# DakeQQ/Text-to-Speech-TTS-ONNX

Hardware: AMD Instinct MI355X
Metric: audio_seconds_per_second (higher is better)
Workload: dtype f32

## Files before the change

text-to-speech-tts-onnx_amd/csrc/gemm_x3d.hip:

```cpp
#include "common.h"
#include "mfma.h"
#include "gemm_epilogue.h"
#include "x3_split.h"
#include "lds_dma.h"
#include <type_traits>
#include <algorithm>

namespace mi {

typedef float f32x4 __attribute__((ext_vector_type(4)));

template <int TW> struct X3dGeom {
    static constexpr int TM = 144, MB = 3;
    static constexpr int KG = TW == 64 ? 2 : 1;
    static constexpr int WNS = KG == 2 ? 2 : 4;
    static constexpr int WNW = TW / WNS, NB = WNW / 16;
#ifndef X3D_S128
#define X3D_S128 1
#endif
    static constexpr int S = TW == 192 ? 1 : TW == 128 ? X3D_S128 : 2;
    static constexpr int WSTEP = TW == 128 ? X3D_S128 : 1;
    static constexpr int R = TW == 64 ? 6 : TW == 128 ? 4 : 3;
    static constexpr int LB = R / S - 1;
    static constexpr int A_PLANE = TM * 64, B_PLANE = TW * 64;
    static constexpr int A_BYTES = 2 * A_PLANE, CH = A_BYTES + 2 * B_PLANE;
    static constexpr int PC = CH / 1024, P = S * PC;
    static constexpr int NHI = (P + 11) / 12, NHIW = P - 12 * (NHI - 1);
    static constexpr int NCB = TW / 64, NRB = 5, BLK = 2176;
    static constexpr int STG = NRB * NCB * BLK * 4, RING = R * CH;
    static constexpr int LNT = RING > STG ? RING : STG;
    static constexpr int SMEM = LNT + 2 * 160 * 4;
    static_assert(SMEM <= 163840, "x3d: LDS");
};

template <int OFF> __device__ __forceinline__ void x3d_lds_rd128(f16x8& d, unsigned a) {
#if defined(__HIP_DEVICE_COMPILE__)
    asm volatile("ds_read_b128 %0, %1 offset:%2" : "=v"(d) : "v"(a), "n"(OFF) : "memory");
#endif
}
template <int OFF, int N> struct X3dRd {
    static __device__ __forceinline__ void go(f16x8 (&dst)[N], unsigned a) {
        X3dRd<OFF, N - 1>::go(reinterpret_cast<f16x8 (&)[N - 1]>(dst), a);
        x3d_lds_rd128<OFF + (N - 1) * 1024>(dst[N - 1], a);
    }
};
template <int OFF> struct X3dRd<OFF, 1> {
    static __device__ __forceinline__ void go(f16x8 (&dst)[1], unsigned a) { x3d_lds_rd128<OFF>(dst[0], a); }
};
template <int N, int I = 0, typename F> __device__ __forceinline__ void x3d_unroll(F&& f) {
    if constexpr (I < N) { f(std::integral_constant<int, I>{}); x3d_unroll<N, I + 1>(f); }
}
template <int TW, bool FOLD, int EPK>
__global__ __launch_bounds__(768) void linear_x3d_kernel(const ConvGemmDev p) {
    using G = X3dGeom<TW>;
    using Frag = f16x8;
    constexpr int MB = G::MB, NB = G::NB;
    __shared__ __attribute__((aligned(1024))) unsigned char smem[G::SMEM];
    (void)smem;
#if defined(__HIP_DEVICE_COMPILE__)
    const int tid = threadIdx.x, lane = tid & 63;
    const int wave = __builtin_amdgcn_readfirstlane(tid >> 6);
    const int per = (int)gridDim.x >> 3;
    const int u = ((int)blockIdx.x & 7) * per + ((int)blockIdx.x >> 3);
    const int RGn = p.Tm, CGn = p.Tn, band = p.RT;
    if (u >= RGn * CGn) return;
    const int bi = u / (band * CGn);
    const int rem = u - bi * band * CGn;
    const int bh = min(band, RGn - bi * band);
    const int cg = rem / bh, rg = bi * band + rem - cg * bh;
    const int m0 = rg * G::TM, n0 = cg * TW;
    const int nch = p.K >> 5;

    const int kg = G::KG == 2 ? wave / 6 : 0;
    const int w6 = G::KG == 2 ? wave - kg * 6 : wave;
    const int wm = w6 / G::WNS, wn = w6 - wm * G::WNS;

    const int bytesA = (int)((long)((p.M + 127) >> 7) * nch * 16384), bytesB = (int)((long)((p.N + 127) >> 7) * nch * 16384);
    const unsigned smem_lds = lds_addr(smem);
    const int voff = lane * 16;
    constexpr int OOB = 0x7fffff00;
    int pc_gbase[G::NHI], pc_cs[G::NHI];
    unsigned pc_lofs[G::NHI];
    __amdgpu_buffer_rsrc_t pc_rs[G::NHI];
#pragma unroll
    for (int i = 0; i < G::NHI; ++i) {
        const int q = wave + 12 * i;
        const int cs = q / G::PC, r = q - cs * G::PC;
        const bool isA = r < 18;
        const int rr = isA ? r : r - 18;
        const int gpp = isA ? 9 : TW / 16;
        const int plane = rr / gpp, g16 = rr - plane * gpp;
        const int row = (isA ? m0 : n0) + 16 * g16;
        pc_cs[i] = cs;
        pc_rs[i] = buf_rsrc(isA ? p.x : p.w3, isA ? bytesA : bytesB);
        pc_gbase[i] = __builtin_amdgcn_readfirstlane((row >> 7) * nch * 16384 + plane * 8192 + (row & 127) * 64);
        pc_lofs[i] = (unsigned)__builtin_amdgcn_readfirstlane(isA ? plane * G::A_PLANE + g16 * 1024 : G::A_BYTES + plane * G::B_PLANE + g16 * 1024);
    }
    const bool hi_wave = wave < G::NHIW;
    auto issue_piece = [&](int t, auto I_) __attribute__((always_inline)) {
        constexpr int i = decltype(I_)::value;
        if constexpr (i < G::NHI) {
            if (i == G::NHI - 1 && !hi_wave) return;
            const int chunk = t * G::S + pc_cs[i];
            const int soff = __builtin_amdgcn_readfirstlane(chunk < nch ? pc_gbase[i] + chunk * 16384 : OOB);
            const unsigned dst = __builtin_amdgcn_readfirstlane(smem_lds + (unsigned)((chunk % G::R) * G::CH) + pc_lofs[i]);
            dma16_buf(pc_rs[i], (int)((unsigned)voff + (unsigned)soff), dst);
        }
    };
    auto issue_batch = [&](int t) __attribute__((always_inline)) {
        x3d_unroll<G::NHI>([&](auto I_) __attribute__((always_inline)) { issue_piece(t, I_); });
    };
    auto wait_batches = [&](auto NB_) __attribute__((always_inline)) {
        constexpr int n = decltype(NB_)::value;
        if (hi_wave) wait_vm<n * G::NHI>(); else wait_vm<n * (G::NHI - 1)>();
    };

    const int fi = lane & 15, fs = lane >> 4;
    const int sig = (0x1320 >> (4 * (fi >> 2))) & 3;
    const unsigned f_lane = (unsigned)((4 * sig + (fi & 3)) * 64 + ((fs ^ sig) << 4));
    const unsigned fa_off = (unsigned)(wm * 48 * 64) + f_lane;
    const unsigned fb_off = (unsigned)(G::A_BYTES + wn * G::WNW * 64) + f_lane;
    Frag a_lo[MB], a_hi[MB], b_lo[NB], b_hi[NB];
    f32x4 acc0[MB][NB], acc1[MB][NB];
#pragma unroll
    for (int i = 0; i < MB; ++i)
#pragma unroll
        for (int j = 0; j < NB; ++j) { acc0[i][j] = f32x4{0.f, 0.f, 0.f, 0.f}; acc1[i][j] = f32x4{0.f, 0.f, 0.f, 0.f}; }
    auto rd_a = [&](unsigned a, auto PL, Frag (&dst)[MB]) __attribute__((always_inline)) {
        constexpr int pl = decltype(PL)::value;
        X3dRd<pl * G::A_PLANE, MB>::go(dst, a);
    };
    auto rd_b = [&](unsigned b, auto PL, Frag (&dst)[NB]) __attribute__((always_inline)) {
        constexpr int pl = decltype(PL)::value;
        X3dRd<pl * G::B_PLANE, NB>::go(dst, b);
    };
    using P0 = std::integral_constant<int, 0>;
    using P1 = std::integral_constant<int, 1>;
    auto mma = [&](const Frag (&a)[MB], const Frag (&b)[NB], f32x4 (&c)[MB][NB]) __attribute__((always_inline)) {
#pragma unroll
        for (int i = 0; i < MB; ++i)
#pragma unroll
            for (int j = 0; j < NB; ++j) c[i][j] = __builtin_amdgcn_mfma_f32_16x16x32_f16(a[i], b[j], c[i][j], 0, 0, 0);
    };
#define X3D_SB() __builtin_amdgcn_sched_barrier(0)

    const int NJ = nch / G::KG;
#pragma unroll
    for (int t = 0; t <= G::LB; ++t) issue_batch(t);
    float* lnt = reinterpret_cast<float*>(smem + G::LNT);
    constexpr bool CONSUMER = FOLD && (EPK == 1 || EPK == 2);
    if constexpr (CONSUMER) {
        if (wave < G::NRB && p.ln_stats_in) {
            float rs, mr;
            ln_rows32(p, (long)p.m_off + m0 + wave * 32, (long)p.m_off + p.M - 1, lane & 31, lane >> 5, rs, mr);
            if (lane < 32) { lnt[wave * 32 + lane] = rs; lnt[160 + wave * 32 + lane] = mr; }
        }
    }
    wait_batches(std::integral_constant<int, G::LB>{});
    __builtin_amdgcn_s_barrier();
    {
        const unsigned s0 = smem_lds + (unsigned)((kg % G::R) * G::CH);
        rd_a(s0 + fa_off, P1{}, a_lo); rd_b(s0 + fb_off, P0{}, b_hi); rd_a(s0 + fa_off, P0{}, a_hi); rd_b(s0 + fb_off, P1{}, b_lo);
    }
    auto chunk = [&](int j, auto BAR_) __attribute__((always_inline)) {
        constexpr bool BAR = decltype(BAR_)::value;
        wait_lgkm<MB + NB>();
        X3D_SB(); mma(a_lo, b_hi, acc1); X3D_SB();
        const int jn = j + 1;
        const int ts = jn / G::WSTEP;
        if constexpr (BAR) {
            wait_batches(std::integral_constant<int, G::LB - 1>{});
            wait_lgkm<0>();
            __builtin_amdgcn_s_barrier();
        }
        const unsigned sn = smem_lds + (unsigned)(((jn * G::KG + kg) % G::R) * G::CH);
        rd_a(sn + fa_off, P1{}, a_lo);
        wait_lgkm<MB>();
        X3D_SB();
        x3d_unroll<MB * NB>([&](auto IDX_) __attribute__((always_inline)) {
            constexpr int idx = decltype(IDX_)::value, i = idx / NB, jj = idx % NB;
            acc0[i][jj] = __builtin_amdgcn_mfma_f32_16x16x32_f16(a_hi[i], b_hi[jj], acc0[i][jj], 0, 0, 0);
            if constexpr (BAR) issue_piece(ts + G::LB, IDX_);
            X3D_SB();
        });
        rd_b(sn + fb_off, P0{}, b_hi);
        X3D_SB(); mma(a_hi, b_lo, acc1); X3D_SB();
        rd_a(sn + fa_off, P0{}, a_hi); rd_b(sn + fb_off, P1{}, b_lo);
    };
    static_assert(G::NHI <= MB * NB, "x3d: a batch's pieces ride on the MFMAs of phase 1");
    for (int j = 0; j < NJ; j += G::WSTEP) {
        if constexpr (G::WSTEP == 2) chunk(j, std::false_type{});
        chunk(j + G::WSTEP - 1, std::true_type{});
    }
#undef X3D_SB
    wait_vm<0>();
    wait_lgkm<0>();
    __builtin_amdgcn_s_barrier();
    if (p.dbg & 4) return;

    float* stg = reinterpret_cast<float*>(smem);
    {
        const int rq = 4 * ((0x1320 >> (4 * (lane >> 4))) & 3);
        const int cq = 4 * ((0x1320 >> (4 * ((lane & 15) >> 2))) & 3) + (lane & 3);
        auto put = [&](bool add) __attribute__((always_inline)) {
#pragma unroll
            for (int i = 0; i < MB; ++i) {
                const int row = wm * 48 + i * 16 + rq;
#pragma unroll
                for (int j = 0; j < NB; ++j) {
                    const int col = wn * G::WNW + j * 16 + cq;
                    float* d = stg + ((row >> 5) * G::NCB + (col >> 6)) * G::BLK + (row & 31) * 64 + (col & 63);
#pragma unroll
                    for (int r = 0; r < 4; ++r) {
                        const float v = __builtin_fmaf(acc1[i][j][r], 0x1p-11f, acc0[i][j][r]);
                        d[r * 64] = add ? d[r * 64] + v : v;
                    }
                }
            }
        };
        if (G::KG == 1 || kg == 0) put(false);
        __syncthreads();
        if constexpr (G::KG == 2) {
            if (kg == 1) put(true);
            __syncthreads();
        }
    }
    const int lr = lane & 31, lk = lane >> 5;
    const int m_end = min(p.M, m0 + G::TM);
    constexpr bool HALVES = EPK == 3 && (G::NRB * G::NCB * G::BLK + 12 * 1024) * 4 <= G::LNT;
    if constexpr (HALVES) {
        float* half_stage = stg + G::NRB * G::NCB * G::BLK;
        for (int u = wave; u < G::NRB * G::NCB * 2; u += 12) {
            const int b = u >> 1, hf = u & 1;
            const int rb = b / G::NCB, cb = b - rb * G::NCB;
            if (m0 + rb * 32 >= m_end) continue;
            const float* blk = stg + b * G::BLK + hf * 32;
            f32x16 h1[1][1];
#pragma unroll
            for (int r = 0; r < 16; ++r) {
                const float t = blk[((r & 3) + 8 * (r >> 2) + 4 * lk) * 64 + lr];
                h1[0][0][r] = (rb == G::NRB - 1 && r >= 8) ? 0.f : t;
            }
            float* st = half_stage + wave * 1024;
            if constexpr (FOLD) gemm_epilogue_resid_ln<float, 1, 1, 2>(h1, p, m0 + rb * 32, n0 + cb * 64 + hf * 32, lr, lk, st, m_end);
            else gemm_epilogue_lds<float, 1, 1, 32, 32>(h1, p, m0, n0, 0, 0, rb, cb * 2 + hf, lr, lk, st, m_end);
        }
        return;
    }
    for (int b = wave; b < G::NRB * G::NCB; b += 12) {
        const int rb = b / G::NCB, cb = b - rb * G::NCB;
        if (m0 + rb * 32 >= m_end) continue;
        float* blk = stg + b * G::BLK;
        float prs[1] = {0.f}, pmr[1] = {0.f};
        if constexpr (CONSUMER) { prs[0] = lnt[rb * 32 + lr]; pmr[0] = lnt[160 + rb * 32 + lr]; }
        f32x16 h[1][2];
#pragma unroll
        for (int j = 0; j < 2; ++j)
#pragma unroll
            for (int r = 0; r < 16; ++r) {
                const float t = blk[((r & 3) + 8 * (r >> 2) + 4 * lk) * 64 + j * 32 + lr];
                h[0][j][r] = (rb == G::NRB - 1 && r >= 8) ? 0.f : t;
            }
        __builtin_amdgcn_fence(__ATOMIC_ACQUIRE, "wavefront");
        __builtin_amdgcn_wave_barrier();
        if constexpr (FOLD) {
            if constexpr (EPK == 1) gemm_epilogue_qkv_lds<float, 1, true, true>(h, p, m0, n0, 0, rb, cb, lr, lk, blk, prs, pmr, m_end);
            else if constexpr (EPK == 2) gemm_epilogue_ln_in<float, 1, 2, 2, true>(h, p, m0 + rb * 32, n0 + cb * 64, lr, lk, blk, prs, pmr, m_end);
            else gemm_epilogue_resid_ln<float, 1, 2, 2>(h, p, m0 + rb * 32, n0 + cb * 64, lr, lk, blk, m_end);
        } else {
            if constexpr (EPK == 1) gemm_epilogue_qkv_lds<float, 1>(h, p, m0, n0, 0, rb, cb, lr, lk, blk, nullptr, nullptr, m_end);
            else if constexpr (EPK == 2) x3p_epilogue_planes<1, 2, 2>(h, p, m0, n0, rb, cb, lr, lk, blk, m_end);
            else gemm_epilogue_lds<float, 1, 2, 32, 64>(h, p, m0, n0, 0, 0, rb, cb, lr, lk, blk, m_end);
        }
    }
#endif
}


bool x3d_plan(const ConvGemmDev& e, int cus, int& tw, int& rgn, int& cgn, int& band) {
    if (!opt(OPT_GEMM_X3D) || e.np != 2 || !e.lds_epi || e.K % 32 != 0 || cus < 8) return false;
    const int nch = e.K / 32;
    double best = 0.0; int btw = 0;
    for (int w : {192, 128, 64}) {
        if (e.N % w != 0) continue;
        if (w != 192 && nch % 2 != 0) continue;
        if (e.epi == EPI_QKV_ROPE && w % 64 != 0) continue;
        const long tiles = (long)((e.M + 143) / 144) * (e.N / w);
        const long rounds = (tiles + cus - 1) / cus;
        const double eff = (double)e.M * e.N / ((double)rounds * cus * 144.0 * w);
        if (eff > best + 1e-9) { best = eff; btw = w; }
    }
    if (!btw || best * 100.0 < (double)opt(OPT_GEMM_X3D_MIN_EFF)) return false;
    tw = btw; rgn = (e.M + 143) / 144; cgn = e.N / btw;
    int ba = 1; double bc = 1e300;
    for (int a = 1; a <= 32; a *= 2) {
        if (a > rgn && a > 1) break;
        const double c = (double)std::min(a, rgn) * 144.0 + (double)std::min(32 / a, cgn) * tw;
        if (c < bc) { bc = c; ba = a; }
    }
    band = std::min(ba, rgn);
    return true;
}

void launch_linear_x3d(const ConvGemmDev& e_in, int tw, int rgn, int cgn, int band, hipStream_t s) {
    ConvGemmDev e = e_in;
    e.Tm = rgn; e.Tn = cgn; e.RT = band;
    const long tiles = (long)rgn * cgn;
    const dim3 grid((unsigned)(((tiles + 7) / 8) * 8));
    const bool fold = e.ln_stats_in || e.ln_stats_out;
    const int epk = e.epi == EPI_QKV_ROPE ? 1 : fold ? (e.ln_stats_in ? 2 : 3) : (e.out_planes ? 2 : 3);
#define X3D_GO(TW_, FOLD_, EPK_, LABEL)                                                                                           \
    do {                                                                                                                          \
        prof_set_kernel("linear_x3d_kernel<" #TW_ ", " LABEL ">", "", "");                                                        \
        hipLaunchKernelGGL((linear_x3d_kernel<TW_, FOLD_, EPK_>), grid, dim3(768), 0, s, e);                                      \
    } while (0)
#define X3D_ROLE(TW_)                                                                                                             \
    do {                                                                                                                          \
        if (fold) { if (epk == 1) X3D_GO(TW_, true, 1, "AdaLN fold, QKV"); else if (epk == 2) X3D_GO(TW_, true, 2, "AdaLN fold, FF1"); else X3D_GO(TW_, true, 3, "AdaLN fold, O / FF2"); } \
        else { if (epk == 1) X3D_GO(TW_, false, 1, "QKV"); else if (epk == 2) X3D_GO(TW_, false, 2, "planes out"); else X3D_GO(TW_, false, 3, "rows out"); } \
    } while (0)
    if (tw == 192) X3D_ROLE(192); else if (tw == 128) X3D_ROLE(128); else X3D_ROLE(64);
#undef X3D_ROLE
#undef X3D_GO
    MI_HIP(hipGetLastError());
}

}
```

text-to-speech-tts-onnx_amd/csrc/options.h:

```cpp
#pragma once
#include <atomic>
#include <shared_mutex>

namespace mi {

#define MI_OPTIONS(X)                                                                                                   \
                                   \
    X(GEMM_BIG_TILE_MIN, "gemm_big_tile_min", "MI355TTS_BIG_TILE_MIN", ENV_INT, 160, STORE, 0, 0)                       \
    X(GEMM_N192_MIN, "gemm_n192_min", nullptr, ENV_INT, 160, STORE, 0, 0)                                               \
    X(GEMM_MID_TILE_MIN, "gemm_mid_tile_min", nullptr, ENV_INT, 160, STORE, 0, 0)                                       \
    X(GEMM_DMA3_K_MIN, "gemm_dma3_k_min", "MI355TTS_DMA3_K_MIN", ENV_INT, 2048, STORE, 0, 0)                            \
    X(GEMM_USE_DMA3, "gemm_use_dma3", "MI355TTS_NO_DMA3_GEMM", ENV_ONE_OFF, 1, BOOL, 0, 1)                              \
    X(GEMM_USE_DMA, "gemm_use_dma", "MI355TTS_NO_DMA_GEMM", ENV_ONE_OFF, 1, BOOL, 0, 1)                                 \
    X(GEMM_BIG_TILES, "gemm_big_tiles", "MI355TTS_NO_BIG_TILES", ENV_ONE_OFF, 1, BOOL, 0, 1)                            \
    X(GEMM_N192, "gemm_n192", "MI355TTS_NO_N192", ENV_ONE_OFF, 1, BOOL, 0, 1)                                           \
    X(GEMM_F32_DMA, "gemm_f32_dma", nullptr, ENV_INT, 1, BOOL, 0, 1)                                                    \
    X(GEMM_RING4, "gemm_ring4", "MI355TTS_NO_RING4", ENV_ONE_OFF, 1, BOOL, 0, 1)                                        \
    X(GEMM_RING4_MAX, "gemm_ring4_max", "MI355TTS_RING4_MAX", ENV_INT, 256, STORE, 0, 0)                                \
    X(GEMM_BUF, "gemm_buf", "MI355TTS_NO_BUF", ENV_ONE_OFF, 1, BOOL, 0, 1)                                              \
    X(GEMM_F32_SMALL, "gemm_f32_small", "MI355TTS_NO_F32_SMALL", ENV_ONE_OFF, 1, BOOL, 0, 1)                            \
    X(GEMM_F32_SMALL_MAX, "gemm_f32_small_max", "MI355TTS_F32_SMALL_MAX", ENV_INT, 1024, STORE, 0, 0)                   \
    X(GEMM_SMALL16_MAX, "gemm_small16_max", "MI355TTS_SMALL16_MAX", ENV_INT, 256, STORE, 0, 0)                          \
    X(GEMM_F32_N64_DMA, nullptr, "MI355TTS_F32_N64_DMA", ENV_INT, 1, STORE, 0, 0)                                       \
    X(GEMM_N64_DMA16, nullptr, "MI355TTS_N64_DMA16", ENV_INT, 0, STORE, 0, 0)  \
    X(GEMM_XCD_ORDER, nullptr, "MI355TTS_XCD_ORDER", ENV_ONE_ON, 0, BOOL, 0, 1)                                         \
    X(GEMM_LDS_EPI, nullptr, "MI355TTS_NO_LDS_EPI", ENV_ONE_OFF, 1, BOOL, 0, 1)                                         \
    X(GEMM_ROW_SPLIT, "gemm_row_split", nullptr, ENV_INT, 1, STORE, 0, 0)  \
     \
    X(GEMM_SK, "gemm_sk", "MI355TTS_SK", ENV_INT, 1, STORE, 0, 0)                                                       \
    X(GEMM_SK_STAGES, "gemm_sk_stages", "MI355TTS_SK_STAGES", ENV_INT, 0, STORE, 0, 0)                                  \
    X(GEMM_SK_ORDER, nullptr, "MI355TTS_SK_ORDER", ENV_INT, -1, STORE, 0, 0)                                            \
     \
     \
    X(GEMM_SK_QKV32, nullptr, "MI355TTS_SK_QKV32", ENV_INT, 0, STORE, 0, 0)                                             \
     \
    X(GEMM_F32_X3, "gemm_f32_x3", "MI355TTS_F32_X3", ENV_INT, 1, STORE, 0, 0)                                           \
    X(GEMM_F32_X3P, "gemm_f32_x3p", "MI355TTS_F32_X3P", ENV_INT, 1, STORE, 0, 0)                                        \
    X(GEMM_F32_PLANES, "gemm_f32_planes", "MI355TTS_F32_PLANES", ENV_INT, 2, REJECT, 2, 3)  \
    X(GEMM_F32_N64_PAIRS, "gemm_f32_n64_pairs", nullptr, ENV_INT, 1, STORE, 0, 0)  \
    X(GEMM_F32_GCONV, "gemm_f32_gconv", nullptr, ENV_INT, 1, STORE, 0, 0)  \
    X(GEMM_X3P_NOALIGN, "gemm_x3p_noalign", "MI355TTS_X3P_NOALIGN", ENV_INT, 0, STORE, 0, 0)  \
    X(GEMM_X3P_GRID, "gemm_x3p_grid", "MI355TTS_X3P_GRID", ENV_INT, 0, STORE, 0, 0)  \
    X(GEMM_X3D, "gemm_x3d", "MI355TTS_X3D", ENV_INT, 1, STORE, 0, 0)                            \
    X(GEMM_X3D_MIN_EFF, "gemm_x3d_min_eff", "MI355TTS_X3D_MIN_EFF", ENV_INT, 90, STORE, 0, 0)  \
       \
    X(GEMM_PH8, "gemm_ph8", "MI355TTS_PH8", ENV_INT, 1, STORE, 0, 0)                                                    \
    X(GEMM_PH8_MIN_TILES, "gemm_ph8_min_tiles", "MI355TTS_PH8_MIN", ENV_INT, 200, STORE, 0, 0)                          \
    X(GEMM_PH8_ORDER, "gemm_ph8_order", "MI355TTS_PH8_ORDER", ENV_INT, 1, STORE, 0, 0)                                  \
     \
    X(GEMM_PH8_SPLIT_MAX, "gemm_ph8_split_max", "MI355TTS_PH8_SPLIT", ENV_INT, 2, CLAMP, 1, 4)                          \
    X(GEMM_PH8_SPLIT_MIN_NK, "gemm_ph8_split_min_nk", nullptr, ENV_INT, 24, STORE, 0, 0)                                \
                                                                            \
    X(GCONV_TWO_TAPS, "gconv_two_taps", "MI355TTS_GCONV2", ENV_ZERO_OFF, 1, BOOL, 0, 1)                                 \
    X(GCONV16, "gconv16", "MI355TTS_GCONV16", ENV_ZERO_OFF, 1, BOOL, 0, 1)                                              \
                                                                                         \
    X(ATTN_F32_X3, "attn_f32_x3", "MI355TTS_ATTN_X3", ENV_INT, 2, CLAMP, 0, 2)                                          \
    X(ATTN_F32_PLANES, "attn_f32_planes", "MI355TTS_ATTN_PLANES", ENV_INT, 2, REJECT, 2, 3)  \
    X(ATTN_SPLIT, "attn_split", "MI355TTS_ATTN_NO_SPLIT", ENV_ONE_OFF, 2, CLAMP, 0, 2)  \
    X(ATTN_XCD_MAP, "attn_xcd_map", nullptr, ENV_INT, 1, BOOL, 0, 1)  \
    X(ATTN_KV_PLANES, "attn_kv_planes", "MI355TTS_ATTN_KVP", ENV_INT, 1, BOOL, 0, 1)  \
    X(ATTN_V_ROWS, nullptr, "MI355TTS_ATTN_V_ROWS", ENV_ZERO_OFF, 1, BOOL, 0, 1)  \
    X(ATTN_LPT, "attn_lpt", "MI355TTS_ATTN_LPT", ENV_INT, 1, BOOL, 0, 1)  \
    X(ATTN_Z_FORCE, "attn_z_force", nullptr, ENV_INT, 0, CLAMP, 0, 4)  \
            \
    X(ATTN_Z, nullptr, "MI355TTS_ATTN_Z", ENV_INT, 4, CLAMP, 1, 4)                                                      \
    X(ATTN_Z16, nullptr, "MI355TTS_ATTN_Z16", ENV_INT, 1, CLAMP, 1, 4)                                                  \
    X(ATTN_CUTS, nullptr, "MI355TTS_ATTN_CUTS", ENV_CUTS, 0, STORE, 0, 0)  \
                                                                                              \
    X(GPT_MFMA_MIN, "gpt_mfma_min", nullptr, ENV_INT, 9, STORE, 0, 0)  \
    X(GPT_MFMA, nullptr, "MI355TTS_GPT_NO_MFMA", ENV_ONE_OFF, 1, BOOL, 0, 1)                                            \
                                                                    \
    X(BIGVGAN_STREAMS, "bigvgan_streams", nullptr, ENV_INT, 3, CLAMP, 1, 3)                                             \
    X(BV_SYNC, nullptr, "MI355TTS_BV_SYNC", ENV_ONE_ON, 0, BOOL, 0, 1)                                                  \
    X(AA_TILE, nullptr, "MI355TTS_AA_TILE", ENV_INT, 8192, STORE, 0, 0)    \
    X(AA_PIPE, nullptr, "MI355TTS_AA_PIPE", ENV_ZERO_OFF, 1, BOOL, 0, 1)                                                \
    X(AA_R, nullptr, "MI355TTS_AA_R", ENV_INT, 16, STORE, 0, 0)  \
    X(AACONV_LDS_MIN, nullptr, "MI355TTS_AACONV_LDS_MIN", ENV_INT, 0, STORE, 0, 0)

#define MI_OPT_ENUM(name, key, env, conv, dflt, policy, lo, hi) OPT_##name,
enum Opt : int { MI_OPTIONS(MI_OPT_ENUM) OPT_COUNT };

extern std::atomic<long> g_opt[OPT_COUNT];
static inline long opt(Opt o) { return g_opt[o].load(std::memory_order_relaxed); }

void options_init();
bool options_set(const char* key, long v);
bool options_get(const char* key, long* v);
struct AttnCuts { int n = 0; int c[3] = {0, 0, 0}; };
const AttnCuts& opt_attn_cuts();

long env_int(const char* name, long dflt);
bool env_first_is(const char* name, char c);

long option_epoch();
void option_epoch_bump();
std::shared_mutex& option_lock();
}
```

Baseline: 41.64.

## Add direct register epilogue for x3d FF1 GEMM at TW=128

Moves the x3d kernel body into a header and builds it twice. The new DIRECT variant, for the FF1/planes-out case at tile width 128, changes the B-fragment LDS layout so each lane's accumulators hold 8 contiguous output columns. Those lanes then apply bias or AdaLN fold, the activation and the fp16 plane split straight from registers to global memory. This skips the LDS staging pass, the block-wide sync and the lds-based epilogue. It is on by default through a new option, and it risks different store coalescing and extra register pressure.

```diff
diff --git a/text-to-speech-tts-onnx_amd/csrc/gemm_x3d.hip b/text-to-speech-tts-onnx_amd/csrc/gemm_x3d.hip
--- a/text-to-speech-tts-onnx_amd/csrc/gemm_x3d.hip
+++ b/text-to-speech-tts-onnx_amd/csrc/gemm_x3d.hip
@@ -3,6 +3,8 @@
 #include "gemm_epilogue.h"
 #include "x3_split.h"
 #include "lds_dma.h"
+#include "x3d_direct.h"
+#include "options.h"
 #include <type_traits>
 #include <algorithm>
 
@@ -50,232 +52,14 @@
 template <int N, int I = 0, typename F> __device__ __forceinline__ void x3d_unroll(F&& f) {
     if constexpr (I < N) { f(std::integral_constant<int, I>{}); x3d_unroll<N, I + 1>(f); }
 }
-template <int TW, bool FOLD, int EPK>
-__global__ __launch_bounds__(768) void linear_x3d_kernel(const ConvGemmDev p) {
-    using G = X3dGeom<TW>;
-    using Frag = f16x8;
-    constexpr int MB = G::MB, NB = G::NB;
-    __shared__ __attribute__((aligned(1024))) unsigned char smem[G::SMEM];
-    (void)smem;
-#if defined(__HIP_DEVICE_COMPILE__)
-    const int tid = threadIdx.x, lane = tid & 63;
-    const int wave = __builtin_amdgcn_readfirstlane(tid >> 6);
-    const int per = (int)gridDim.x >> 3;
-    const int u = ((int)blockIdx.x & 7) * per + ((int)blockIdx.x >> 3);
-    const int RGn = p.Tm, CGn = p.Tn, band = p.RT;
-    if (u >= RGn * CGn) return;
-    const int bi = u / (band * CGn);
-    const int rem = u - bi * band * CGn;
-    const int bh = min(band, RGn - bi * band);
-    const int cg = rem / bh, rg = bi * band + rem - cg * bh;
-    const int m0 = rg * G::TM, n0 = cg * TW;
-    const int nch = p.K >> 5;
-
-    const int kg = G::KG == 2 ? wave / 6 : 0;
-    const int w6 = G::KG == 2 ? wave - kg * 6 : wave;
-    const int wm = w6 / G::WNS, wn = w6 - wm * G::WNS;
-
-    const int bytesA = (int)((long)((p.M + 127) >> 7) * nch * 16384), bytesB = (int)((long)((p.N + 127) >> 7) * nch * 16384);
-    const unsigned smem_lds = lds_addr(smem);
-    const int voff = lane * 16;
-    constexpr int OOB = 0x7fffff00;
-    int pc_gbase[G::NHI], pc_cs[G::NHI];
-    unsigned pc_lofs[G::NHI];
-    __amdgpu_buffer_rsrc_t pc_rs[G::NHI];
-#pragma unroll
-    for (int i = 0; i < G::NHI; ++i) {
-        const int q = wave + 12 * i;
-        const int cs = q / G::PC, r = q - cs * G::PC;
-        const bool isA = r < 18;
-        const int rr = isA ? r : r - 18;
-        const int gpp = isA ? 9 : TW / 16;
-        const int plane = rr / gpp, g16 = rr - plane * gpp;
-        const int row = (isA ? m0 : n0) + 16 * g16;
-        pc_cs[i] = cs;
-        pc_rs[i] = buf_rsrc(isA ? p.x : p.w3, isA ? bytesA : bytesB);
-        pc_gbase[i] = __builtin_amdgcn_readfirstlane((row >> 7) * nch * 16384 + plane * 8192 + (row & 127) * 64);
-        pc_lofs[i] = (unsigned)__builtin_amdgcn_readfirstlane(isA ? plane * G::A_PLANE + g16 * 1024 : G::A_BYTES + plane * G::B_PLANE + g16 * 1024);
-    }
-    const bool hi_wave = wave < G::NHIW;
-    auto issue_piece = [&](int t, auto I_) __attribute__((always_inline)) {
-        constexpr int i = decltype(I_)::value;
-        if constexpr (i < G::NHI) {
-            if (i == G::NHI - 1 && !hi_wave) return;
-            const int chunk = t * G::S + pc_cs[i];
-            const int soff = __builtin_amdgcn_readfirstlane(chunk < nch ? pc_gbase[i] + chunk * 16384 : OOB);
-            const unsigned dst = __builtin_amdgcn_readfirstlane(smem_lds + (unsigned)((chunk % G::R) * G::CH) + pc_lofs[i]);
-            dma16_buf(pc_rs[i], (int)((unsigned)voff + (unsigned)soff), dst);
-        }
-    };
-    auto issue_batch = [&](int t) __attribute__((always_inline)) {
-        x3d_unroll<G::NHI>([&](auto I_) __attribute__((always_inline)) { issue_piece(t, I_); });
-    };
-    auto wait_batches = [&](auto NB_) __attribute__((always_inline)) {
-        constexpr int n = decltype(NB_)::value;
-        if (hi_wave) wait_vm<n * G::NHI>(); else wait_vm<n * (G::NHI - 1)>();
-    };
-
-    const int fi = lane & 15, fs = lane >> 4;
-    const int sig = (0x1320 >> (4 * (fi >> 2))) & 3;
-    const unsigned f_lane = (unsigned)((4 * sig + (fi & 3)) * 64 + ((fs ^ sig) << 4));
-    const unsigned fa_off = (unsigned)(wm * 48 * 64) + f_lane;
-    const unsigned fb_off = (unsigned)(G::A_BYTES + wn * G::WNW * 64) + f_lane;
-    Frag a_lo[MB], a_hi[MB], b_lo[NB], b_hi[NB];
-    f32x4 acc0[MB][NB], acc1[MB][NB];
-#pragma unroll
-    for (int i = 0; i < MB; ++i)
-#pragma unroll
-        for (int j = 0; j < NB; ++j) { acc0[i][j] = f32x4{0.f, 0.f, 0.f, 0.f}; acc1[i][j] = f32x4{0.f, 0.f, 0.f, 0.f}; }
-    auto rd_a = [&](unsigned a, auto PL, Frag (&dst)[MB]) __attribute__((always_inline)) {
-        constexpr int pl = decltype(PL)::value;
-        X3dRd<pl * G::A_PLANE, MB>::go(dst, a);
-    };
-    auto rd_b = [&](unsigned b, auto PL, Frag (&dst)[NB]) __attribute__((always_inline)) {
-        constexpr int pl = decltype(PL)::value;
-        X3dRd<pl * G::B_PLANE, NB>::go(dst, b);
-    };
-    using P0 = std::integral_constant<int, 0>;
-    using P1 = std::integral_constant<int, 1>;
-    auto mma = [&](const Frag (&a)[MB], const Frag (&b)[NB], f32x4 (&c)[MB][NB]) __attribute__((always_inline)) {
-#pragma unroll
-        for (int i = 0; i < MB; ++i)
-#pragma unroll
-            for (int j = 0; j < NB; ++j) c[i][j] = __builtin_amdgcn_mfma_f32_16x16x32_f16(a[i], b[j], c[i][j], 0, 0, 0);
-    };
-#define X3D_SB() __builtin_amdgcn_sched_barrier(0)
-
-    const int NJ = nch / G::KG;
-#pragma unroll
-    for (int t = 0; t <= G::LB; ++t) issue_batch(t);
-    float* lnt = reinterpret_cast<float*>(smem + G::LNT);
-    constexpr bool CONSUMER = FOLD && (EPK == 1 || EPK == 2);
-    if constexpr (CONSUMER) {
-        if (wave < G::NRB && p.ln_stats_in) {
-            float rs, mr;
-            ln_rows32(p, (long)p.m_off + m0 + wave * 32, (long)p.m_off + p.M - 1, lane & 31, lane >> 5, rs, mr);
-            if (lane < 32) { lnt[wave * 32 + lane] = rs; lnt[160 + wave * 32 + lane] = mr; }
-        }
-    }
-    wait_batches(std::integral_constant<int, G::LB>{});
-    __builtin_amdgcn_s_barrier();
-    {
-        const unsigned s0 = smem_lds + (unsigned)((kg % G::R) * G::CH);
-        rd_a(s0 + fa_off, P1{}, a_lo); rd_b(s0 + fb_off, P0{}, b_hi); rd_a(s0 + fa_off, P0{}, a_hi); rd_b(s0 + fb_off, P1{}, b_lo);
-    }
-    auto chunk = [&](int j, auto BAR_) __attribute__((always_inline)) {
-        constexpr bool BAR = decltype(BAR_)::value;
-        wait_lgkm<MB + NB>();
-        X3D_SB(); mma(a_lo, b_hi, acc1); X3D_SB();
-        const int jn = j + 1;
-        const int ts = jn / G::WSTEP;
-        if constexpr (BAR) {
-            wait_batches(std::integral_constant<int, G::LB - 1>{});
-            wait_lgkm<0>();
-            __builtin_amdgcn_s_barrier();
-        }
-        const unsigned sn = smem_lds + (unsigned)(((jn * G::KG + kg) % G::R) * G::CH);
-        rd_a(sn + fa_off, P1{}, a_lo);
-        wait_lgkm<MB>();
-        X3D_SB();
-        x3d_unroll<MB * NB>([&](auto IDX_) __attribute__((always_inline)) {
-            constexpr int idx = decltype(IDX_)::value, i = idx / NB, jj = idx % NB;
-            acc0[i][jj] = __builtin_amdgcn_mfma_f32_16x16x32_f16(a_hi[i], b_hi[jj], acc0[i][jj], 0, 0, 0);
-            if constexpr (BAR) issue_piece(ts + G::LB, IDX_);
-            X3D_SB();
-        });
-        rd_b(sn + fb_off, P0{}, b_hi);
-        X3D_SB(); mma(a_hi, b_lo, acc1); X3D_SB();
-        rd_a(sn + fa_off, P0{}, a_hi); rd_b(sn + fb_off, P1{}, b_lo);
-    };
-    static_assert(G::NHI <= MB * NB, "x3d: a batch's pieces ride on the MFMAs of phase 1");
-    for (int j = 0; j < NJ; j += G::WSTEP) {
-        if constexpr (G::WSTEP == 2) chunk(j, std::false_type{});
-        chunk(j + G::WSTEP - 1, std::true_type{});
-    }
-#undef X3D_SB
-    wait_vm<0>();
-    wait_lgkm<0>();
-    __builtin_amdgcn_s_barrier();
-    if (p.dbg & 4) return;
-
-    float* stg = reinterpret_cast<float*>(smem);
-    {
-        const int rq = 4 * ((0x1320 >> (4 * (lane >> 4))) & 3);
-        const int cq = 4 * ((0x1320 >> (4 * ((lane & 15) >> 2))) & 3) + (lane & 3);
-        auto put = [&](bool add) __attribute__((always_inline)) {
-#pragma unroll
-            for (int i = 0; i < MB; ++i) {
-                const int row = wm * 48 + i * 16 + rq;
-#pragma unroll
-                for (int j = 0; j < NB; ++j) {
-                    const int col = wn * G::WNW + j * 16 + cq;
-                    float* d = stg + ((row >> 5) * G::NCB + (col >> 6)) * G::BLK + (row & 31) * 64 + (col & 63);
-#pragma unroll
-                    for (int r = 0; r < 4; ++r) {
-                        const float v = __builtin_fmaf(acc1[i][j][r], 0x1p-11f, acc0[i][j][r]);
-                        d[r * 64] = add ? d[r * 64] + v : v;
-                    }
-                }
-            }
-        };
-        if (G::KG == 1 || kg == 0) put(false);
-        __syncthreads();
-        if constexpr (G::KG == 2) {
-            if (kg == 1) put(true);
-            __syncthreads();
-        }
-    }
-    const int lr = lane & 31, lk = lane >> 5;
-    const int m_end = min(p.M, m0 + G::TM);
-    constexpr bool HALVES = EPK == 3 && (G::NRB * G::NCB * G::BLK + 12 * 1024) * 4 <= G::LNT;
-    if constexpr (HALVES) {
-        float* half_stage = stg + G::NRB * G::NCB * G::BLK;
-        for (int u = wave; u < G::NRB * G::NCB * 2; u += 12) {
-            const int b = u >> 1, hf = u & 1;
-            const int rb = b / G::NCB, cb = b - rb * G::NCB;
-            if (m0 + rb * 32 >= m_end) continue;
-            const float* blk = stg + b * G::BLK + hf * 32;
-            f32x16 h1[1][1];
-#pragma unroll
-            for (int r = 0; r < 16; ++r) {
-                const float t = blk[((r & 3) + 8 * (r >> 2) + 4 * lk) * 64 + lr];
-                h1[0][0][r] = (rb == G::NRB - 1 && r >= 8) ? 0.f : t;
-            }
-            float* st = half_stage + wave * 1024;
-            if constexpr (FOLD) gemm_epilogue_resid_ln<float, 1, 1, 2>(h1, p, m0 + rb * 32, n0 + cb * 64 + hf * 32, lr, lk, st, m_end);
-            else gemm_epilogue_lds<float, 1, 1, 32, 32>(h1, p, m0, n0, 0, 0, rb, cb * 2 + hf, lr, lk, st, m_end);
-        }
-        return;
-    }
-    for (int b = wave; b < G::NRB * G::NCB; b += 12) {
-        const int rb = b / G::NCB, cb = b - rb * G::NCB;
-        if (m0 + rb * 32 >= m_end) continue;
-        float* blk = stg + b * G::BLK;
-        float prs[1] = {0.f}, pmr[1] = {0.f};
-        if constexpr (CONSUMER) { prs[0] = lnt[rb * 32 + lr]; pmr[0] = lnt[160 + rb * 32 + lr]; }
-        f32x16 h[1][2];
-#pragma unroll
-        for (int j = 0; j < 2; ++j)
-#pragma unroll
-            for (int r = 0; r < 16; ++r) {
-                const float t = blk[((r & 3) + 8 * (r >> 2) + 4 * lk) * 64 + j * 32 + lr];
-                h[0][j][r] = (rb == G::NRB - 1 && r >= 8) ? 0.f : t;
-            }
-        __builtin_amdgcn_fence(__ATOMIC_ACQUIRE, "wavefront");
-        __builtin_amdgcn_wave_barrier();
-        if constexpr (FOLD) {
-            if constexpr (EPK == 1) gemm_epilogue_qkv_lds<float, 1, true, true>(h, p, m0, n0, 0, rb, cb, lr, lk, blk, prs, pmr, m_end);
-            else if constexpr (EPK == 2) gemm_epilogue_ln_in<float, 1, 2, 2, true>(h, p, m0 + rb * 32, n0 + cb * 64, lr, lk, blk, prs, pmr, m_end);
-            else gemm_epilogue_resid_ln<float, 1, 2, 2>(h, p, m0 + rb * 32, n0 + cb * 64, lr, lk, blk, m_end);
-        } else {
-            if constexpr (EPK == 1) gemm_epilogue_qkv_lds<float, 1>(h, p, m0, n0, 0, rb, cb, lr, lk, blk, nullptr, nullptr, m_end);
-            else if constexpr (EPK == 2) x3p_epilogue_planes<1, 2, 2>(h, p, m0, n0, rb, cb, lr, lk, blk, m_end);
-            else gemm_epilogue_lds<float, 1, 2, 32, 64>(h, p, m0, n0, 0, 0, rb, cb, lr, lk, blk, m_end);
-        }
-    }
-#endif
+#define X3D_KERNEL_DIRECT false
+#include "gemm_x3d_kernel.h"
+#undef X3D_KERNEL_DIRECT
+namespace direct {
+#define X3D_KERNEL_DIRECT true
+#include "gemm_x3d_kernel.h"
+#undef X3D_KERNEL_DIRECT
 }
-
 
 bool x3d_plan(const ConvGemmDev& e, int cus, int& tw, int& rgn, int& cgn, int& band) {
     if (!opt(OPT_GEMM_X3D) || e.np != 2 || !e.lds_epi || e.K % 32 != 0 || cus < 8) return false;
@@ -319,6 +103,17 @@
         if (fold) { if (epk == 1) X3D_GO(TW_, true, 1, "AdaLN fold, QKV"); else if (epk == 2) X3D_GO(TW_, true, 2, "AdaLN fold, FF1"); else X3D_GO(TW_, true, 3, "AdaLN fold, O / FF2"); } \
         else { if (epk == 1) X3D_GO(TW_, false, 1, "QKV"); else if (epk == 2) X3D_GO(TW_, false, 2, "planes out"); else X3D_GO(TW_, false, 3, "rows out"); } \
     } while (0)
+#define X3D_GO_DIRECT(TW_, FOLD_, EPK_, LABEL)                                                                                    \
+    do {                                                                                                                          \
+        prof_set_kernel("linear_x3d_kernel<" #TW_ ", " LABEL ">", "", "");                                                        \
+        hipLaunchKernelGGL((direct::linear_x3d_kernel<TW_, FOLD_, EPK_>), grid, dim3(768), 0, s, e);                              \
+    } while (0)
+    if (opt(OPT_GEMM_X3D_DIRECT_EPI) && tw == 128 && epk == 2) {
+        if (fold) X3D_GO_DIRECT(128, true, 2, "AdaLN fold, FF1"); else X3D_GO_DIRECT(128, false, 2, "planes out");
+        MI_HIP(hipGetLastError());
+        return;
+    }
+#undef X3D_GO_DIRECT
     if (tw == 192) X3D_ROLE(192); else if (tw == 128) X3D_ROLE(128); else X3D_ROLE(64);
 #undef X3D_ROLE
 #undef X3D_GO
diff --git a/text-to-speech-tts-onnx_amd/csrc/gemm_x3d_kernel.h b/text-to-speech-tts-onnx_amd/csrc/gemm_x3d_kernel.h
--- /dev/null
+++ b/text-to-speech-tts-onnx_amd/csrc/gemm_x3d_kernel.h
@@ -0,0 +1,270 @@
+template <int TW, bool FOLD, int EPK>
+__global__ __launch_bounds__(768) void linear_x3d_kernel(const ConvGemmDev p) {
+    constexpr bool DIRECT = X3D_KERNEL_DIRECT;
+    using G = X3dGeom<TW>;
+    using Frag = f16x8;
+    constexpr int MB = G::MB, NB = G::NB;
+    static_assert(!DIRECT || (NB == 2 && EPK == 2 && G::KG == 1), "x3d: the direct epilogue is FF1 at TW = 128");
+    __shared__ __attribute__((aligned(1024))) unsigned char smem[G::SMEM];
+    (void)smem;
+#if defined(__HIP_DEVICE_COMPILE__)
+    const int tid = threadIdx.x, lane = tid & 63;
+    const int wave = __builtin_amdgcn_readfirstlane(tid >> 6);
+    const int per = (int)gridDim.x >> 3;
+    const int u = ((int)blockIdx.x & 7) * per + ((int)blockIdx.x >> 3);
+    const int RGn = p.Tm, CGn = p.Tn, band = p.RT;
+    if (u >= RGn * CGn) return;
+    const int bi = u / (band * CGn);
+    const int rem = u - bi * band * CGn;
+    const int bh = min(band, RGn - bi * band);
+    const int cg = rem / bh, rg = bi * band + rem - cg * bh;
+    const int m0 = rg * G::TM, n0 = cg * TW;
+    const int nch = p.K >> 5;
+
+    const int kg = G::KG == 2 ? wave / 6 : 0;
+    const int w6 = G::KG == 2 ? wave - kg * 6 : wave;
+    const int wm = w6 / G::WNS, wn = w6 - wm * G::WNS;
+
+    const int bytesA = (int)((long)((p.M + 127) >> 7) * nch * 16384), bytesB = (int)((long)((p.N + 127) >> 7) * nch * 16384);
+    const unsigned smem_lds = lds_addr(smem);
+    const int voff = lane * 16;
+    constexpr int OOB = 0x7fffff00;
+    int pc_gbase[G::NHI], pc_cs[G::NHI];
+    unsigned pc_lofs[G::NHI];
+    __amdgpu_buffer_rsrc_t pc_rs[G::NHI];
+#pragma unroll
+    for (int i = 0; i < G::NHI; ++i) {
+        const int q = wave + 12 * i;
+        const int cs = q / G::PC, r = q - cs * G::PC;
+        const bool isA = r < 18;
+        const int rr = isA ? r : r - 18;
+        const int gpp = isA ? 9 : TW / 16;
+        const int plane = rr / gpp, g16 = rr - plane * gpp;
+        const int row = (isA ? m0 : n0) + 16 * g16;
+        pc_cs[i] = cs;
+        pc_rs[i] = buf_rsrc(isA ? p.x : p.w3, isA ? bytesA : bytesB);
+        pc_gbase[i] = __builtin_amdgcn_readfirstlane((row >> 7) * nch * 16384 + plane * 8192 + (row & 127) * 64);
+        pc_lofs[i] = (unsigned)__builtin_amdgcn_readfirstlane(isA ? plane * G::A_PLANE + g16 * 1024 : G::A_BYTES + plane * G::B_PLANE + g16 * 1024);
+    }
+    const bool hi_wave = wave < G::NHIW;
+    auto issue_piece = [&](int t, auto I_) __attribute__((always_inline)) {
+        constexpr int i = decltype(I_)::value;
+        if constexpr (i < G::NHI) {
+            if (i == G::NHI - 1 && !hi_wave) return;
+            const int chunk = t * G::S + pc_cs[i];
+            const int soff = __builtin_amdgcn_readfirstlane(chunk < nch ? pc_gbase[i] + chunk * 16384 : OOB);
+            const unsigned dst = __builtin_amdgcn_readfirstlane(smem_lds + (unsigned)((chunk % G::R) * G::CH) + pc_lofs[i]);
+            dma16_buf(pc_rs[i], (int)((unsigned)voff + (unsigned)soff), dst);
+        }
+    };
+    auto issue_batch = [&](int t) __attribute__((always_inline)) {
+        x3d_unroll<G::NHI>([&](auto I_) __attribute__((always_inline)) { issue_piece(t, I_); });
+    };
+    auto wait_batches = [&](auto NB_) __attribute__((always_inline)) {
+        constexpr int n = decltype(NB_)::value;
+        if (hi_wave) wait_vm<n * G::NHI>(); else wait_vm<n * (G::NHI - 1)>();
+    };
+
+    const int fi = lane & 15, fs = lane >> 4;
+    const int sig = (0x1320 >> (4 * (fi >> 2))) & 3;
+    const unsigned f_lane = (unsigned)((4 * sig + (fi & 3)) * 64 + ((fs ^ sig) << 4));
+    const unsigned fa_off = (unsigned)(wm * 48 * 64) + f_lane;
+    const int dq = fi >> 2;
+    const unsigned fb_lane = DIRECT ? (unsigned)((dq >> 1) * 1024 + (8 * (dq & 1) + (fi & 3)) * 64 + ((fs ^ (2 * (dq & 1))) << 4)) : f_lane;
+    const unsigned fb_off = (unsigned)(G::A_BYTES + wn * G::WNW * 64) + fb_lane;
+    const unsigned fb_t1 = (unsigned)(256 + ((fs ^ (2 * (dq & 1) + 1)) - (fs ^ (2 * (dq & 1)))) * 16);
+    Frag a_lo[MB], a_hi[MB], b_lo[NB], b_hi[NB];
+    f32x4 acc0[MB][NB], acc1[MB][NB];
+#pragma unroll
+    for (int i = 0; i < MB; ++i)
+#pragma unroll
+        for (int j = 0; j < NB; ++j) { acc0[i][j] = f32x4{0.f, 0.f, 0.f, 0.f}; acc1[i][j] = f32x4{0.f, 0.f, 0.f, 0.f}; }
+    auto rd_a = [&](unsigned a, auto PL, Frag (&dst)[MB]) __attribute__((always_inline)) {
+        constexpr int pl = decltype(PL)::value;
+        X3dRd<pl * G::A_PLANE, MB>::go(dst, a);
+    };
+    auto rd_b = [&](unsigned b, auto PL, Frag (&dst)[NB]) __attribute__((always_inline)) {
+        constexpr int pl = decltype(PL)::value;
+        if constexpr (DIRECT) { x3d_lds_rd128<pl * G::B_PLANE>(dst[0], b); x3d_lds_rd128<pl * G::B_PLANE>(dst[1], b + fb_t1); }
+        else X3dRd<pl * G::B_PLANE, NB>::go(dst, b);
+    };
+    auto mfma = [&](const Frag& a, const Frag& b, const f32x4& c) __attribute__((always_inline)) -> f32x4 {
+        if constexpr (DIRECT) return __builtin_amdgcn_mfma_f32_16x16x32_f16(b, a, c, 0, 0, 0);
+        else return __builtin_amdgcn_mfma_f32_16x16x32_f16(a, b, c, 0, 0, 0);
+    };
+    using P0 = std::integral_constant<int, 0>;
+    using P1 = std::integral_constant<int, 1>;
+    auto mma = [&](const Frag (&a)[MB], const Frag (&b)[NB], f32x4 (&c)[MB][NB]) __attribute__((always_inline)) {
+#pragma unroll
+        for (int i = 0; i < MB; ++i)
+#pragma unroll
+            for (int j = 0; j < NB; ++j) c[i][j] = mfma(a[i], b[j], c[i][j]);
+    };
+#define X3D_SB() __builtin_amdgcn_sched_barrier(0)
+
+    const int NJ = nch / G::KG;
+    const int d_col = n0 + wn * G::WNW + 8 * (lane >> 4);
+    const int d_trow = wm * 48 + 4 * sig + (fi & 3);
+    float e_a[8], e_b[8];
+    (void)e_a; (void)e_b; (void)d_col; (void)d_trow;
+    if constexpr (DIRECT) {
+        if constexpr (FOLD) { x3d_load8(p.ln_p + d_col, e_a); x3d_load8(p.ln_c + d_col, e_b); }
+        else x3d_load8(p.bias ? p.bias + d_col : (const float*)p.x, e_a);
+    }
+#pragma unroll
+    for (int t = 0; t <= G::LB; ++t) issue_batch(t);
+    float* lnt = reinterpret_cast<float*>(smem + G::LNT);
+    constexpr bool CONSUMER = FOLD && (EPK == 1 || EPK == 2);
+    if constexpr (CONSUMER) {
+        if (wave < G::NRB && p.ln_stats_in) {
+            float rs, mr;
+            ln_rows32(p, (long)p.m_off + m0 + wave * 32, (long)p.m_off + p.M - 1, lane & 31, lane >> 5, rs, mr);
+            if (lane < 32) { lnt[wave * 32 + lane] = rs; lnt[160 + wave * 32 + lane] = mr; }
+        }
+    }
+    wait_batches(std::integral_constant<int, G::LB>{});
+    __builtin_amdgcn_s_barrier();
+    {
+        const unsigned s0 = smem_lds + (unsigned)((kg % G::R) * G::CH);
+        rd_a(s0 + fa_off, P1{}, a_lo); rd_b(s0 + fb_off, P0{}, b_hi); rd_a(s0 + fa_off, P0{}, a_hi); rd_b(s0 + fb_off, P1{}, b_lo);
+    }
+    auto chunk = [&](int j, auto BAR_) __attribute__((always_inline)) {
+        constexpr bool BAR = decltype(BAR_)::value;
+        wait_lgkm<MB + NB>();
+        X3D_SB(); mma(a_lo, b_hi, acc1); X3D_SB();
+        const int jn = j + 1;
+        const int ts = jn / G::WSTEP;
+        if constexpr (BAR) {
+            wait_batches(std::integral_constant<int, G::LB - 1>{});
+            wait_lgkm<0>();
+            __builtin_amdgcn_s_barrier();
+        }
+        const unsigned sn = smem_lds + (unsigned)(((jn * G::KG + kg) % G::R) * G::CH);
+        rd_a(sn + fa_off, P1{}, a_lo);
+        wait_lgkm<MB>();
+        X3D_SB();
+        x3d_unroll<MB * NB>([&](auto IDX_) __attribute__((always_inline)) {
+            constexpr int idx = decltype(IDX_)::value, i = idx / NB, jj = idx % NB;
+            acc0[i][jj] = mfma(a_hi[i], b_hi[jj], acc0[i][jj]);
+            if constexpr (BAR) issue_piece(ts + G::LB, IDX_);
+            X3D_SB();
+        });
+        rd_b(sn + fb_off, P0{}, b_hi);
+        X3D_SB(); mma(a_hi, b_lo, acc1); X3D_SB();
+        rd_a(sn + fa_off, P0{}, a_hi); rd_b(sn + fb_off, P1{}, b_lo);
+    };
+    static_assert(G::NHI <= MB * NB, "x3d: a batch's pieces ride on the MFMAs of phase 1");
+    for (int j = 0; j < NJ; j += G::WSTEP) {
+        if constexpr (G::WSTEP == 2) chunk(j, std::false_type{});
+        chunk(j + G::WSTEP - 1, std::true_type{});
+    }
+#undef X3D_SB
+    wait_vm<0>();
+    wait_lgkm<0>();
+    __builtin_amdgcn_s_barrier();
+    if (p.dbg & 4) return;
+
+    if constexpr (DIRECT) {
+        const int m_end = min(p.M, m0 + G::TM);
+        float v[MB][8];
+#pragma unroll
+        for (int i = 0; i < MB; ++i)
+#pragma unroll
+            for (int j = 0; j < 2; ++j)
+#pragma unroll
+                for (int r = 0; r < 4; ++r) v[i][4 * j + r] = __builtin_fmaf(acc1[i][j][r], 0x1p-11f, acc0[i][j][r]);
+        unsigned sat = 0;
+        if constexpr (!FOLD) {
+            if (!p.bias) {
+#pragma unroll
+                for (int q = 0; q < 8; ++q) e_a[q] = 0.f;
+            }
+        }
+#pragma unroll
+        for (int i = 0; i < MB; ++i) {
+            const int tr = d_trow + 16 * i, m = m0 + tr;
+            float rs = 0.f, mr = 0.f;
+            if constexpr (FOLD) { rs = lnt[tr]; mr = lnt[160 + tr]; }
+            x3d_direct_planes<FOLD>(p, v[i], m, d_col, m < m_end, rs, mr, e_a, e_b, sat);
+        }
+        sat_publish(p.sat, sat);
+        return;
+    }
+
+    float* stg = reinterpret_cast<float*>(smem);
+    {
+        const int rq = 4 * ((0x1320 >> (4 * (lane >> 4))) & 3);
+        const int cq = 4 * ((0x1320 >> (4 * ((lane & 15) >> 2))) & 3) + (lane & 3);
+        auto put = [&](bool add) __attribute__((always_inline)) {
+#pragma unroll
+            for (int i = 0; i < MB; ++i) {
+                const int row = wm * 48 + i * 16 + rq;
+#pragma unroll
+                for (int j = 0; j < NB; ++j) {
+                    const int col = wn * G::WNW + j * 16 + cq;
+                    float* d = stg + ((row >> 5) * G::NCB + (col >> 6)) * G::BLK + (row & 31) * 64 + (col & 63);
+#pragma unroll
+                    for (int r = 0; r < 4; ++r) {
+                        const float v = __builtin_fmaf(acc1[i][j][r], 0x1p-11f, acc0[i][j][r]);
+                        d[r * 64] = add ? d[r * 64] + v : v;
+                    }
+                }
+            }
+        };
+        if (G::KG == 1 || kg == 0) put(false);
+        __syncthreads();
+        if constexpr (G::KG == 2) {
+            if (kg == 1) put(true);
+            __syncthreads();
+        }
+    }
+    const int lr = lane & 31, lk = lane >> 5;
+    const int m_end = min(p.M, m0 + G::TM);
+    constexpr bool HALVES = EPK == 3 && (G::NRB * G::NCB * G::BLK + 12 * 1024) * 4 <= G::LNT;
+    if constexpr (HALVES) {
+        float* half_stage = stg + G::NRB * G::NCB * G::BLK;
+        for (int u = wave; u < G::NRB * G::NCB * 2; u += 12) {
+            const int b = u >> 1, hf = u & 1;
+            const int rb = b / G::NCB, cb = b - rb * G::NCB;
+            if (m0 + rb * 32 >= m_end) continue;
+            const float* blk = stg + b * G::BLK + hf * 32;
+            f32x16 h1[1][1];
+#pragma unroll
+            for (int r = 0; r < 16; ++r) {
+                const float t = blk[((r & 3) + 8 * (r >> 2) + 4 * lk) * 64 + lr];
+                h1[0][0][r] = (rb == G::NRB - 1 && r >= 8) ? 0.f : t;
+            }
+            float* st = half_stage + wave * 1024;
+            if constexpr (FOLD) gemm_epilogue_resid_ln<float, 1, 1, 2>(h1, p, m0 + rb * 32, n0 + cb * 64 + hf * 32, lr, lk, st, m_end);
+            else gemm_epilogue_lds<float, 1, 1, 32, 32>(h1, p, m0, n0, 0, 0, rb, cb * 2 + hf, lr, lk, st, m_end);
+        }
+        return;
+    }
+    for (int b = wave; b < G::NRB * G::NCB; b += 12) {
+        const int rb = b / G::NCB, cb = b - rb * G::NCB;
+        if (m0 + rb * 32 >= m_end) continue;
+        float* blk = stg + b * G::BLK;
+        float prs[1] = {0.f}, pmr[1] = {0.f};
+        if constexpr (CONSUMER) { prs[0] = lnt[rb * 32 + lr]; pmr[0] = lnt[160 + rb * 32 + lr]; }
+        f32x16 h[1][2];
+#pragma unroll
+        for (int j = 0; j < 2; ++j)
+#pragma unroll
+            for (int r = 0; r < 16; ++r) {
+                const float t = blk[((r & 3) + 8 * (r >> 2) + 4 * lk) * 64 + j * 32 + lr];
+                h[0][j][r] = (rb == G::NRB - 1 && r >= 8) ? 0.f : t;
+            }
+        __builtin_amdgcn_fence(__ATOMIC_ACQUIRE, "wavefront");
+        __builtin_amdgcn_wave_barrier();
+        if constexpr (FOLD) {
+            if constexpr (EPK == 1) gemm_epilogue_qkv_lds<float, 1, true, true>(h, p, m0, n0, 0, rb, cb, lr, lk, blk, prs, pmr, m_end);
+            else if constexpr (EPK == 2) gemm_epilogue_ln_in<float, 1, 2, 2, true>(h, p, m0 + rb * 32, n0 + cb * 64, lr, lk, blk, prs, pmr, m_end);
+            else gemm_epilogue_resid_ln<float, 1, 2, 2>(h, p, m0 + rb * 32, n0 + cb * 64, lr, lk, blk, m_end);
+        } else {
+            if constexpr (EPK == 1) gemm_epilogue_qkv_lds<float, 1>(h, p, m0, n0, 0, rb, cb, lr, lk, blk, nullptr, nullptr, m_end);
+            else if constexpr (EPK == 2) x3p_epilogue_planes<1, 2, 2>(h, p, m0, n0, rb, cb, lr, lk, blk, m_end);
+            else gemm_epilogue_lds<float, 1, 2, 32, 64>(h, p, m0, n0, 0, 0, rb, cb, lr, lk, blk, m_end);
+        }
+    }
+#endif
+}
diff --git a/text-to-speech-tts-onnx_amd/csrc/options.h b/text-to-speech-tts-onnx_amd/csrc/options.h
--- a/text-to-speech-tts-onnx_amd/csrc/options.h
+++ b/text-to-speech-tts-onnx_amd/csrc/options.h
@@ -43,6 +43,7 @@
     X(GEMM_X3P_GRID, "gemm_x3p_grid", "MI355TTS_X3P_GRID", ENV_INT, 0, STORE, 0, 0)  \
     X(GEMM_X3D, "gemm_x3d", "MI355TTS_X3D", ENV_INT, 1, STORE, 0, 0)                            \
     X(GEMM_X3D_MIN_EFF, "gemm_x3d_min_eff", "MI355TTS_X3D_MIN_EFF", ENV_INT, 90, STORE, 0, 0)  \
+    X(GEMM_X3D_DIRECT_EPI, nullptr, "MI355TTS_X3D_DIRECT_EPI", ENV_ZERO_OFF, 1, BOOL, 0, 1)  \
        \
     X(GEMM_PH8, "gemm_ph8", "MI355TTS_PH8", ENV_INT, 1, STORE, 0, 0)                                                    \
     X(GEMM_PH8_MIN_TILES, "gemm_ph8_min_tiles", "MI355TTS_PH8_MIN", ENV_INT, 200, STORE, 0, 0)                          \
diff --git a/text-to-speech-tts-onnx_amd/csrc/x3d_direct.h b/text-to-speech-tts-onnx_amd/csrc/x3d_direct.h
--- /dev/null
+++ b/text-to-speech-tts-onnx_amd/csrc/x3d_direct.h
@@ -0,0 +1,43 @@
+#pragma once
+#include "gemm_epilogue.h"
+
+namespace mi {
+
+__device__ __forceinline__ void x3d_hop(float (&x)[8]) {
+#if defined(__HIP_DEVICE_COMPILE__)
+#pragma unroll
+    for (int q = 0; q < 8; ++q) asm volatile("" : "+v"(x[q]));
+#endif
+}
+__device__ __forceinline__ void x3d_load8(const float* src, float (&d)[8]) {
+    const float4 a = *reinterpret_cast<const float4*>(src), b = *reinterpret_cast<const float4*>(src + 4);
+    d[0] = a.x; d[1] = a.y; d[2] = a.z; d[3] = a.w; d[4] = b.x; d[5] = b.y; d[6] = b.z; d[7] = b.w;
+}
+__device__ __forceinline__ void x3d_store_planes(void* planes, int N, int m, int col, bool ok, const float (&x)[8], unsigned& sat) {
+    u32x4 pl[2];
+    unsigned s = 0;
+    xnp_split8_sat<2>(x, pl, s);
+    if (ok) {
+        sat |= s;
+        unsigned char* dst = (unsigned char*)planes + x3p_slot_offset(m, col >> 3, N >> 5, 2);
+        *reinterpret_cast<u32x4*>(dst) = pl[0];
+        *reinterpret_cast<u32x4*>(dst + X3P_PLANE) = pl[1];
+    }
+}
+
+template <bool FOLD>
+__device__ __forceinline__ void x3d_direct_planes(const ConvGemmDev& p, float (&x)[8], int m, int col, bool ok, float rs, float mr,
+                                                  const float (&pv)[8], const float (&cv)[8], unsigned& sat) {
+    if constexpr (FOLD) {
+#pragma unroll
+        for (int q = 0; q < 8; ++q) x[q] = __builtin_fmaf(rs, x[q], __builtin_fmaf(-mr, pv[q], cv[q]));
+    } else {
+#pragma unroll
+        for (int q = 0; q < 8; ++q) x[q] = x[q] + pv[q];
+    }
+    ln_act8<float>(x, p.act);
+    x3d_hop(x);
+    x3d_store_planes(p.out_planes, p.N, m, col, ok, x, sat);
+}
+
+}
```

After: 41.92 (median of 6 runs). Within noise of the previous version (+0.7%).
